# HybridRobotics/ilqr-iterative-tasks

Measured on AMD Instinct MI355X. Metric: batched iLQR iterations/s (n=6,m=2,N=20), higher is better.
Workload: dtype f64

## Files before the change

ilqr_iterative_tasks_amd/csrc/i2lqr_abi.hip:

```cpp
#include <hip/hip_runtime.h>

#include <atomic>
#include <cmath>
#include <cstdarg>
#include <cstdio>
#include <cstdlib>
#include <cstring>
#include <mutex>
#include <new>
#include <unordered_set>

#include "../../include/i2lqr.h"
#include "i2lqr_devcfg.hpp"
#include "i2lqr_geometry.hpp"
#include "i2lqr_group.h"
#include "i2lqr_host.hpp"
#include "i2lqr_kernels.h"
#include "i2lqr_lane12.h"
#include "i2lqr_rccl.hpp"
#include "i2lqr_select.hpp"
#include "i2lqr_wave_ls.h"
#include "i2lqr_wave_box.h"
#include "i2lqr_wave_obs.h"

// ... 107 lines not shown
                (long long)(rec & 0xfffffff));
  }
#else
  (void)stream;
#endif
  return rc;
}
}

struct i2lqr_handle {
  i2lqr_config cfg;
  int lanes;
  size_t lds_bytes;
  int device;
  void* ws = nullptr;
  int64_t ws_bytes = 0;
  int64_t compact_min_batch = -1;
  int opt_defer = -1, opt_reroll = -1, opt_lds_steps = -1, opt_merge = -1, opt_ckpt = -1, opt_stagger = -1;
  int wave_tail = -1;
  int opt_pair = -1;
  int opt_two_x = -1;
  int opt_chunk_step = -1;
  int opt_fuse = -1;
  int opt_final_round = -1;
  int opt_first_chunk = -1;
  int opt_fstep = -1;
  int opt_group = -1;
  int opt_spec = -1;
  int opt_group_ws = -1;
  int opt_group_overlap = -1;
  int opt_obs = 0;
  i2lqr::StateBox box;
  int opt_ls = 0;
  int opt_group_fixed = -1;
  struct Epilogue {
    const int32_t* qfun;
    int outer_iter, max_relax_iter;
    void* cost_it;
    void* part;
    int64_t* best_idx;
    void* best_cost;
    bool fused;
  };
  static constexpr unsigned kTickets = 16;
  unsigned* ticket = nullptr;
  std::atomic<unsigned> ticket_next{0};
  hipEvent_t ev_ready = nullptr, ev_side_done = nullptr;
  bool side_pending = false;
  DeviceGeometry geo;
};

namespace {
thread_local i2lqr_handle::Epilogue* t_epi = nullptr;
}

namespace {

enum FusedKernel { K_WAVE, K_WAVE_LS, K_WAVE_OBS, K_WAVE_BOX, K_GROUP, K_GROUP16, K_GROUP_WS, K_SPEC, K_SPEC16, K_QUAD, K_INVALID };
constexpr int64_t kAutoGroupBatch = 1024;
constexpr int64_t kAutoSpecBatch = 12288;

FusedKernel select_fused(const i2lqr_handle* h, int64_t B, bool early_exit, const char** why) {
  static const char* none = "";
  if (!why) why = &none;
  if (h->box.on()) {
    if (h->opt_group == 8 || h->opt_group == 16) {
// ... 110 lines not shown
  static constexpr int n = Sys::n, m = Sys::m, LANES = 64;
  using Cfg = DevCfg<T, n, m>;

  static size_t lds_bytes(int N) { return (size_t)Layout<Sys>(N).total * sizeof(T) * (64 / LANES); }
  static size_t fstep_lds_bytes(int N) {
    return (size_t)Layout<Sys>(N, true).total * sizeof(T) * (64 / LANES);
  }
  static constexpr bool kHasFstep = Sys::n <= 6;
  static unsigned grid(int64_t B) { return (unsigned)((B + (64 / LANES) - 1) / (64 / LANES)); }

  static int prepare(i2lqr_handle* h) {
    h->lanes = LANES;
    h->lds_bytes = lds_bytes(h->cfg.N);
    if (h->lds_bytes > h->geo.max_dyn_lds)
      return fail(I2LQR_ERR_UNSUPPORTED, "horizon %d needs %zu B of LDS per wavefront (> %zu KiB)",
                  h->cfg.N, h->lds_bytes, h->geo.max_dyn_lds / 1024);
    if (h->lds_bytes > h->geo.default_dyn_lds)
      for (const void* kernel :
           {(const void*)k_iterate<T, Sys, LANES, false>, (const void*)k_iterate<T, Sys, LANES, true>,
            (const void*)k_backward<T, Sys, LANES, false>, (const void*)k_backward<T, Sys, LANES, true>,
            (const void*)k_forward<T, Sys, LANES, false>, (const void*)k_forward<T, Sys, LANES, true>,
            (const void*)k_rollout<T, Sys, LANES, false>, (const void*)k_rollout<T, Sys, LANES, true>})
        HIP_TRY(hipFuncSetAttribute(kernel, hipFuncAttributeMaxDynamicSharedMemorySize,
                                    (int)h->lds_bytes));
    return I2LQR_OK;
  }

  static int iterate(i2lqr_handle* h, int64_t B, int n_iters, int early_exit, void* X, void* U,
                     const void* x_term, void* lamb, const void* obs, void* cost, void* K, void* k,
                     int32_t* iters, int32_t* status, hipStream_t s) {
    const Cfg c = make_dev_cfg<T, n, m>(h->cfg);
    IterArgs<T> a = iter_args<T>(B, n_iters, early_exit, X, U, x_term, lamb, obs, cost, K, k, iters,
                                 status);
#ifdef I2LQR_STAMPS
    a.dbg = (unsigned long long*)h->ws;
#endif
    const char* why = "";
    const FusedKernel fk = select_fused(h, B, early_exit != 0, &why);
    if (t_epi && (fk == K_GROUP || fk == K_GROUP16 || fk == K_GROUP_WS)) {
      a.qfun = t_epi->qfun;
      a.outer_iter = t_epi->outer_iter;
      a.max_relax_iter = t_epi->max_relax_iter;
      a.cost_it = (T*)t_epi->cost_it;
      if (t_epi->best_idx) {
        a.pick_part = (MinPair<T>*)t_epi->part;
        a.pick_ticket = h->ticket + h->ticket_next.fetch_add(1, std::memory_order_relaxed) %
                                        i2lqr_handle::kTickets;
        a.best_idx = t_epi->best_idx;
        a.best_cost = (T*)t_epi->best_cost;
      }
      t_epi->fused = true;
    }
    switch (fk) {
      case K_INVALID:
        return fail(I2LQR_ERR_UNSUPPORTED, "%s", why);
      case K_SPEC:
      case K_SPEC16:
        if constexpr (m == 2 && n + m <= 8) {
          HIP_TRY(group_spec_iterate<T>(h->cfg, a, s, fk == K_SPEC16 ? 16 : 8));
          return I2LQR_OK;
        }
        break;
      case K_GROUP:
        if constexpr (m == 2 && n + m <= 8) {
          HIP_TRY(group_iterate<T>(h->cfg, a, s));
          return I2LQR_OK;
// ... 48 lines not shown
    const int64_t waves_per_cu = (grid(B) + h->geo.cus - 1) / h->geo.cus;
    const bool fstep = kHasFstep && lds_f <= h->geo.default_dyn_lds &&
                       (h->opt_fstep >= 0 ? h->opt_fstep != 0
                                          : waves_per_cu * lds_f <= h->geo.lds_per_cu - 10 * 1024);
    if constexpr (kHasFstep) {
      if (fstep) {
        with_weights(c.flags, [&](auto W) {
          hipLaunchKernelGGL((k_iterate<T, Sys, LANES, W, true>), dim3(grid(B)), dim3(64), lds_f, s, c, a);
        });
        HIP_TRY(hipGetLastError());
        return I2LQR_OK;
      }
    }
    with_weights(c.flags, [&](auto W) {
      hipLaunchKernelGGL((k_iterate<T, Sys, LANES, W>), dim3(grid(B)), dim3(64), h->lds_bytes, s, c, a);
    });
    HIP_TRY(hipGetLastError());
    return I2LQR_OK;
  }
  static int names_pair(i2lqr_handle*, int64_t, int) { return 0; }
  static int solve_chained(i2lqr_handle* h, int64_t L, int k, void* X, void* U, const void* x_term,
                           void* lamb, const void* obs, void* cost, void* K, void* kk, int32_t* iters,
                           int32_t* status, hipStream_t s) {
    if constexpr (m == 2 && n + m <= 8) {
      if (h->opt_spec == 0 || h->opt_group == 8 || h->opt_group == 64 ||
          !group_spec_chain_supported(h->cfg, L))
        return fail(I2LQR_ERR_UNSUPPORTED, "chains run on the sixteen-lane speculative kernel: a "
                    "bicycle plant with Q = R = 0, at most %lld chains, a horizon whose three-wavefront "
                    "buffers fit a CU's LDS (solve the chain steps one after the other instead)",
                    (long long)h->geo.scaled(512));
      IterArgs<T> a = iter_args<T>(L, h->cfg.max_iter, 1, X, U, x_term, lamb, obs, cost, K, kk, iters,
                                   status);
      a.chain_len = k;
      HIP_TRY(group_spec_chain<T>(h->cfg, a, s));
      return I2LQR_OK;
    }
    return fail(I2LQR_ERR_UNSUPPORTED, "chains are built for the m = 2 plants");
  }
  static int rollout(i2lqr_handle* h, int64_t B, void* X, void* U, const void* x_term, void* cost,
                     hipStream_t s) {
    const Cfg c = make_dev_cfg<T, n, m>(h->cfg);
    with_weights(c.flags, [&](auto W) {
      hipLaunchKernelGGL((k_rollout<T, Sys, LANES, W>), dim3(grid(B)), dim3(64), h->lds_bytes, s, c,
                         B, (T*)X, (T*)U, (const T*)x_term, (T*)cost);
    });
    HIP_TRY(hipGetLastError());
    return I2LQR_OK;
  }
  static int backward(i2lqr_handle* h, int64_t B, const void* X, const void* U, const void* x_term,
                      const void* lamb, const void* obs, void* K, void* k, hipStream_t s) {
    const Cfg c = make_dev_cfg<T, n, m>(h->cfg);
    with_weights(c.flags, [&](auto W) {
      hipLaunchKernelGGL((k_backward<T, Sys, LANES, W>), dim3(grid(B)), dim3(64), h->lds_bytes, s, c,
                         B, (const T*)X, (const T*)U, (const T*)x_term, (const T*)lamb,
                         (const T*)obs, (T*)K, (T*)k);
    });
    HIP_TRY(hipGetLastError());
    return I2LQR_OK;
  }
  static int forward(i2lqr_handle* h, int64_t B, const void* X, const void* U, const void* x_term,
                     const void* K, const void* k, void* Xn, void* Un, void* cost_new,
                     hipStream_t s) {
    const Cfg c = make_dev_cfg<T, n, m>(h->cfg);
    with_weights(c.flags, [&](auto W) {
      hipLaunchKernelGGL((k_forward<T, Sys, LANES, W>), dim3(grid(B)), dim3(64), h->lds_bytes, s, c,
                         B, (const T*)X, (const T*)U, (const T*)x_term, (const T*)K, (const T*)k,
// ... 248 lines not shown
      a.cp.user_tiled = TILED ? 1 : 0;
      a.cp.orig = orig;
      if (dst) a.cp.dst = *dst;
      a.cp.count_out = count_out;
      a.cp.usr = usr;
    };
    int round = 0;
    int cur = 0;
    const bool only_chunk = len >= max_iter;
    plan_exit(a0, true, nullptr, only_chunk ? nullptr : &cv.set[cur], cv.count + round);
    launch_iterate<TILED>(h->geo, c, a0, B, s, h->opt_pair);
    done += len;
    const unsigned cgrid = (unsigned)((B + 255) / 256);
    bool src_user = true;
    const int32_t* count_in = nullptr;
    LaneSet<T> src = usr;
    const int final_round = (!spec_tail || wave_tail <= 0) ? 0
        : (h->opt_final_round >= 0 ? h->opt_final_round : kFinalRound);
    while (done < max_iter) {
      int32_t* const count = cv.count + round;
      if (!fused)
        hipLaunchKernelGGL((k_lane_compact<T, TILED>), dim3(cgrid), dim3(256), 0, s, n, m, N, src,
                           src_user ? 1 : 0, count_in, cv.set[cur], count, usr, c.trap);
      const LaneSet<T>& w = cv.set[cur];
      const bool tail_ran = wave_tail > 0 && done >= 4;
      const bool last_round = final_round > 0 && round + 1 >= final_round && tail_ran;
      if (tail_ran) {
        using WL = Launch<T, Sys>;
        const size_t lds_f = WL::fstep_lds_bytes(N);
        IterArgs<T> t = iter_args<T>(B, max_iter, 1, w.X, w.U, w.x_term, w.lamb, w.obs, w.cost, w.K,
                                     w.k, w.iters, w.status);
        t.count = count; t.count_max = last_round ? (int)B : wave_tail; t.max_total = max_iter;
        t.set_stride = B;
        if (spec_tail) {
          t.orig = w.orig;
          t.out_X = usr.X; t.out_U = usr.U; t.out_K = usr.K; t.out_k = usr.k;
          t.out_lamb = usr.lamb; t.out_cost = usr.cost;
          t.out_iters = usr.iters; t.out_status = usr.status;
          t.out_B = usr.B; t.out_tiled = TILED ? 1 : 0;
          if constexpr (m == 2 && n + m <= 8) HIP_TRY(group_spec_tail<T>(h->cfg, t, s));
        } else if (WL::kHasFstep && lds_f <= h->geo.default_dyn_lds) {
          if constexpr (WL::kHasFstep) {
            with_weights(c.flags, [&](auto W) {
              hipLaunchKernelGGL((k_iterate<T, Sys, 64, W, true, true>), dim3(wave_tail), dim3(64),
                                 lds_f, s, c, t);
            });
          }
        }
      }
      if (last_round && spec_tail && tail_ran) {
        src_user = true;
        break;
      }
      len = done < 12 ? step : done;
      if (done + len > max_iter || round + 2 >= kMaxRounds) len = max_iter - done;
      LaneArgs<T> a = a0;
      set_io(a, len, 1, w);
      a.K = nullptr; a.k = nullptr;
      a.count = count; a.resume = 1;
      plan_exit(a, false, w.orig, done + len >= max_iter ? nullptr : &cv.set[cur ^ 1],
                cv.count + round + 1);
      LaneArgs<T> ap = a;
      ap.ckpt = 0;
      ap.merge = h->opt_merge >= 0 ? h->opt_merge : 0;
      ap.reroll = h->opt_reroll >= 0 ? h->opt_reroll : 0;
      const unsigned pair_max = pair_max_grid(h->geo);
// ... 506 lines not shown
  return B % 64 == 0 ? I2LQR_LAYOUT_BATCH_TILED : I2LQR_LAYOUT_BATCH_MINOR;
}

int i2lqr_set_compaction(i2lqr_handle* h, int64_t min_batch) {
  if (!h) return fail(I2LQR_ERR_INVALID, "null handle");
  if (h->cfg.layout == I2LQR_LAYOUT_PROBLEM_MAJOR && min_batch > 0)
    return fail(I2LQR_ERR_UNSUPPORTED, "compaction applies to the batch-minor / batch-tiled layouts");
  h->compact_min_batch = min_batch < 0 ? -1 : min_batch;
  return I2LQR_OK;
}

int i2lqr_set_option(i2lqr_handle* h, const char* name, int64_t value) {
  if (!h || !name) return fail(I2LQR_ERR_INVALID, "null handle or option name");
  if (value < -1 || value > 0x7fffffff) return fail(I2LQR_ERR_INVALID, "option value out of range");
  const int v = (int)value;
  if (!strcmp(name, "defer_states")) h->opt_defer = v < 0 ? -1 : (v != 0);
  else if (!strcmp(name, "reroll_nominal")) h->opt_reroll = v < 0 ? -1 : (v != 0);
  else if (!strcmp(name, "lds_gain_steps")) h->opt_lds_steps = v;
  else if (!strcmp(name, "merge_inputs")) h->opt_merge = v < 0 ? -1 : (v != 0);
  else if (!strcmp(name, "checkpoint_states")) h->opt_ckpt = v < 0 ? -1 : (v != 0);
  else if (!strcmp(name, "stagger")) h->opt_stagger = v;
  else if (!strcmp(name, "per_step_jacobians")) h->opt_fstep = v < 0 ? -1 : (v != 0);
  else if (!strcmp(name, "wave_tail")) h->wave_tail = v < 0 ? -1 : (v > 65536 ? 65536 : v);
  else if (!strcmp(name, "first_chunk")) h->opt_first_chunk = v < 1 ? -1 : (v > 1024 ? 1024 : v);
  else if (!strcmp(name, "helper_wavefront")) h->opt_pair = v < 0 ? -1 : (v != 0);
  else if (!strcmp(name, "state_buffers")) h->opt_two_x = v < 0 ? -1 : (v != 0);
  else if (!strcmp(name, "chunk_step")) h->opt_chunk_step = v < 1 ? -1 : (v > 1024 ? 1024 : v);
  else if (!strcmp(name, "fused_compaction")) h->opt_fuse = v < 0 ? -1 : (v != 0);
  else if (!strcmp(name, "final_round")) h->opt_final_round = v < 0 ? -1 : (v > 20 ? 20 : v);
  else if (!strcmp(name, "speculate")) h->opt_spec = v < 0 ? -1 : (v != 0);
  else if (!strcmp(name, "group_workspace")) h->opt_group_ws = v < 0 ? -1 : (v != 0);
  else if (!strcmp(name, "group_overlap")) h->opt_group_overlap = v < 0 ? -1 : (v != 0);
  else if (!strcmp(name, "group_fixed_horizon")) h->opt_group_fixed = v < 0 ? -1 : (v != 0);
  else if (!strcmp(name, "debug_self_test")) {
#ifdef I2LQR_DEBUG
    unsigned long long* w = i2lqr::debug_trap_word();
    double* buf = nullptr;
    HIP_TRY(hipMalloc((void**)&buf, 8 * sizeof(double)));
    hipLaunchKernelGGL(k_debug_self_test, dim3(1), dim3(64), 0, (hipStream_t)0, buf, w);
    const int rc = debug_check(I2LQR_OK, nullptr);
    (void)hipFree(buf);
    return rc;
#else
    return fail(I2LQR_ERR_UNSUPPORTED, "\"debug_self_test\" exists in the index-checked debug build "
                "only (make -C ilqr_iterative_tasks_amd/csrc debug)");
#endif
  }
  else if (!strcmp(name, "line_search")) {
    if (v != -1 && v != 0 && v != 1 && v != 2 && v != 4 && v != 8)
      return fail(I2LQR_ERR_INVALID, "\"line_search\" is 2, 4 or 8 step sizes, or -1 / 0 / 1 (off)");
    if (v > 1 && h->cfg.layout != I2LQR_LAYOUT_PROBLEM_MAJOR)
      return fail(I2LQR_ERR_UNSUPPORTED, "\"line_search\" is built for the problem-major layout (the "
                  "one-problem-per-wavefront kernel)");
    h->opt_ls = v > 1 ? v : 0;
  }
  else if (!strcmp(name, "obstacles")) {
    if (v > I2LQR_MAX_OBSTACLES)
      return fail(I2LQR_ERR_INVALID, "\"obstacles\" is 2 ... %d records per problem, or -1 / 0 / 1 "
                  "(off: one record)", I2LQR_MAX_OBSTACLES);
    if (v > 1 && h->cfg.layout != I2LQR_LAYOUT_PROBLEM_MAJOR)
      return fail(I2LQR_ERR_UNSUPPORTED, "\"obstacles\" is built for the problem-major layout (the "
                  "one-problem-per-wavefront kernel)");
    h->opt_obs = v > 1 ? v : 0;
  }
  else if (!strcmp(name, "group_lanes")) {
    if (v != -1 && v != 8 && v != 16 && v != 64)
// ... 619 lines not shown
```

ilqr_iterative_tasks_amd/csrc/i2lqr_group.hpp:

```cpp
#pragma once
#include <hip/hip_runtime.h>
#include <stdint.h>

#include "i2lqr_systems.hpp"
#include "i2lqr_wave.hpp"

namespace i2lqr {

constexpr int kGroup = 8;
constexpr int kGroupsPerWave = 64 / kGroup;

template <class Sys> struct GroupPattern {
  static constexpr int n = Sys::n, m = Sys::m, W = n + m, NV = Sys::NVAR;
  static constexpr int dt_row(int b) {
    for (int i = 2; i < n; i++)
      if (i != b && Sys::pat(i, b) == 2) return i;
    return -1;
  }
  static constexpr bool column_ok(int b) {
    int extra = 0;
    for (int i = 0; i < n; i++) {
      const int code = Sys::pat(i, b);
      if (i < 2) {
        if (code == 2) return false;
// ... 215 lines not shown
      const T f = code == 2 ? c.dt : jv[code >= 3 ? code - 3 : 0];
      acc = first ? f * v : t_fma(f, v, acc);
      first = false;
    }
  }

  __device__ __forceinline__ T rollout(int XUo, int TRo, const T (&xT)[n]) const {
    T x[n], u[m], xn[n], tr[NT];
#pragma unroll
    for (int i = 0; i < n; i++) x[i] = S[XUo + i];
    const int N = loop_N();
    for (int t = 0; t < N; t++) {
#pragma unroll
      for (int a = 0; a < m; a++) u[a] = clip(S[XUo + t * W + n + a], -c.u_max[a], c.u_max[a]);
#pragma unroll
      for (int a = 0; a < m; a++) S[XUo + t * W + n + a] = u[a];
      Sys::trig(x, tr);
#pragma unroll
      for (int q = 0; q < NT; q++) S[TRo + t * NT + q] = tr[q];
      Sys::step_tr(c, x, u, tr, xn);
#pragma unroll
      for (int i = 0; i < n; i++) S[XUo + (t + 1) * W + i] = xn[i];
#pragma unroll
      for (int i = 0; i < n; i++) x[i] = xn[i];
    }
    Sys::trig(x, tr);
#pragma unroll
    for (int q = 0; q < NT; q++) S[TRo + N * NT + q] = tr[q];
    const T cost = terminal_cost(x, xT);
    wave_sync();
    return cost;
  }

  __device__ __forceinline__ void prep(int XUo, int TRo, const T (&ob)[6], T pa, T pb, int first,
                                       int stride) const {
    const bool has_ob = ob[5] >= T(0);
    const int opt = has_ob ? (int)ob[5] : 0;
    const T spd_y = opt == 1 ? ob[4] : T(0), spd_x = opt == 2 ? ob[4] : T(0);
    const int rounds = (N + stride) / stride;
    for (int r = 0; r < rounds; r++) {
      const int t0 = first + r * stride;
      const int t = t0 < N ? t0 : N;
      const int ts = t0 < N ? t0 : N - 1;
      T* Rs = rec(ts);
      {
        T xe[n], tr[NT], u[m], jv[NV];
#pragma unroll
        for (int i = 0; i < n; i++) xe[i] = S[XUo + (ts + 1) * W + i];
#pragma unroll
        for (int a = 0; a < m; a++) u[a] = S[XUo + ts * W + n + a];
#pragma unroll
        for (int q = 0; q < NT; q++) tr[q] = S[TRo + (ts + 1) * NT + q];
        Sys::jac_var(c, xe, u, tr, jv);
#pragma unroll
        for (int q = 0; q < NV; q++) Rs[GL::R_JV + q] = jv[q];
#pragma unroll
        for (int a = 0; a < m; a++) {
          T e_hi, e_lo;
          if (sizeof(T) == 8 && c.fast_barrier) {
            e_hi = t_exp_bounded(c.ctrl_q2 * (u[a] - c.u_max[a]));
            e_lo = c.ctrl_c[a] * t_rcp(e_hi);
          } else {
            e_hi = t_exp(c.ctrl_q2 * (u[a] - c.u_max[a]));
            e_lo = t_exp(c.ctrl_q2 * (-c.u_max[a] - u[a]));
          }
          Rs[GL::R_LU + a] = c.ctrl_q12 * e_hi - c.ctrl_q12 * e_lo;
          Rs[GL::R_LUU + a] = c.ctrl_q122 * e_hi +
                              c.ctrl_q122 * e_lo;
        }
      }
      T* R = rec(t);
      R[GL::R_ZERO] = T(0);
      R[GL::R_ONE] = T(1);
      const T px = S[XUo + t * W + 0], py = S[XUo + t * W + 1];
      const T dz = opt == 2 ? px - (ob[0] - T(t) * spd_x) : px - ob[0];
      const T dy = opt == 1 ? py - (ob[1] + T(t) * spd_y) : py - ob[1];
      const T h = T(1) + c.safety_margin - (dz * pa * dz + dy * pb * dy);
      const T hd0 = T(-2) * pa * dz, hd1 = T(-2) * pb * dy;
      const T e = t_exp(c.obs_q2 * h);
      const T c1 = c.obs_q12 * e, c2 = c.obs_q122 * e;
      R[GL::R_OB + 0] = has_ob ? c1 * hd0 : T(0);
      R[GL::R_OB + 1] = has_ob ? c1 * hd1 : T(0);
      R[GL::R_OB + 2] = has_ob ? c2 * (hd0 * hd0) : T(0);
      R[GL::R_OB + 3] = has_ob ? c2 * (hd0 * hd1) : T(0);
      R[GL::R_OB + 4] = has_ob ? c2 * (hd1 * hd1) : T(0);
    }
    wave_sync();
    ws_publish();
  }

  __device__ __forceinline__ void quu_inverse(const T (&Quu)[m * m], T lamb, T (&inv)[m * m]) const {
    static_assert(m == 2, "the eight-lane kernel is written for m == 2 plants");
    t_quu_inverse2(Quu, lamb, inv);
  }

  template <bool GENERAL>
  __device__ __forceinline__ bool backward(int XUo, const T (&xT)[n], T lamb, bool commit) const {
    if constexpr (G == 16) return backward_row<GENERAL>(XUo, xT, lamb, commit);
    bool bad = false;
    T va[n];
    {
      const T* Rn = rec(N);
      T dx[n];
#pragma unroll
      for (int i = 0; i < n; i++) dx[i] = S[XUo + N * W + i] - xT[i];
#pragma unroll
      for (int i = 0; i < n; i++) {
        T vxx = T(0), vx = T(0);
#pragma unroll
        for (int r = 0; r < n; r++) {
          const T q = T(2) * Qt[i * n + r];
          vxx = (g == r) ? q : vxx;
          vx += q * dx[r];
        }
        va[i] = (g == n) ? vx : vxx;
      }
      va[0] += Rn[off_l0];
      va[1] += Rn[off_l1];
// ... 114 lines not shown
        for (int b = 0; b < m; b++) acc = t_fma(Quu[a * m + b], kc[b], acc);
        qk[a] = acc;
      }
#pragma unroll
      for (int i = 0; i < n; i++) {
        T acc = T(0);
#pragma unroll
        for (int a = 0; a < m; a++) acc = t_fma(kr[a][i], qk[a], acc);
        va[i] = h[i] - acc;
      }
      STAMP_END(5);
    };
    int t = N - 1;
    if constexpr (I2LQR_GROUP_UNROLL >= 4) {
      for (; t >= 3; t -= 4) {
        step(t, ra, rb);
        step(t - 1, rb, ra);
        step(t - 2, ra, rb);
        step(t - 3, rb, ra);
      }
    }
    for (; t >= 1; t -= 2) {
      step(t, ra, rb);
      step(t - 1, rb, ra);
    }
    if (t == 0) step(0, ra, rb);
    ws_publish();
    return bad;
  }

  template <bool GENERAL>
  __device__ __forceinline__ bool backward_row(int XUo, const T (&xT)[n], T lamb, bool commit) const {
    T vb[n];
    terminal_base(XUo, xT, vb);
    return backward_row_from<GENERAL>(vb, lamb, commit);
  }
  __device__ __forceinline__ void terminal_base(int XUo, const T (&xT)[n], T (&vb)[n]) const {
    T dx[n];
#pragma unroll
    for (int i = 0; i < n; i++) dx[i] = S[XUo + N * W + i] - xT[i];
    const int gq = g < n ? g : 0;
#pragma unroll
    for (int i = 0; i < n; i++) {
      T vx = T(0);
#pragma unroll
      for (int r = 0; r < n; r++) vx += (T(2) * Qt[i * n + r]) * dx[r];
      const T vxx = T(2) * Qt[i * n + gq];
      vb[i] = (g == n) ? vx : (g < n ? vxx : T(0));
    }
  }
  template <bool GENERAL>
  __device__ __forceinline__ bool backward_row_from(const T (&vb)[n], T lamb, bool commit) const {
    static_assert(GL::KW > n + 1, "the padding word of a gain row takes the stores of idle lanes");
    bool bad = false;
    T va[n];
    {
      const T* Rn = rec(N);
#pragma unroll
      for (int i = 0; i < n; i++) va[i] = vb[i];
      va[0] += Rn[off_l0];
      va[1] += Rn[off_l1];
    }
    const int gcol = (commit && g <= n) ? g : GL::KW - 1;
    T cdr[n];
#pragma unroll
    for (int r = 0; r < n; r++) cdr[r] = (rsrc == r) ? cdt : T(0);
    struct Rec { T jv[NV], luu[m], c0, c1, l0, l1, lrow[m]; };
    Rec ra, rb;
    constexpr bool FIXED = NH > 0 && !GENERAL;
    const T* const R0 = rec(0);
    const T *pc0 = R0, *pc1 = R0, *pl0 = R0, *pl1 = R0, *plu[m];
#pragma unroll
    for (int a = 0; a < m; a++) plu[a] = R0;
    if constexpr (FIXED) {
      pc0 = R0 + off_c0; pc1 = R0 + off_c1; pl0 = R0 + off_l0; pl1 = R0 + off_l1;
#pragma unroll
      for (int a = 0; a < m; a++) plu[a] = R0 + off_lu[a];
    }
    auto load_record = [&](int t, Rec& r) __attribute__((always_inline)) {
      if constexpr (FIXED) {
        const int o = t * GL::RW;
// ... 317 lines not shown
  }
};

__device__ __forceinline__ int idx_div(int e, int d, float rcp_d) {
  int q = (int)((float)e * rcp_d);
  const int r = e - q * d;
  q += (r >= d) ? 1 : 0;
  q -= (r < 0) ? 1 : 0;
  return q;
}

template <class T, class Sys, int H, bool WS, int G, int NH>
__device__ __forceinline__ void group_iterate_body(const DevCfg<T, Sys::n, Sys::m>& c,
                                                   const IterArgs<T>& a, T* ws) {
  static_assert(!(WS && H > 1), "the workspace form runs without helper wavefronts");
  constexpr int n = Sys::n, m = Sys::m, W = n + m;
#ifdef I2LQR_STAMPS
  constexpr bool OVL = false;
#else
  constexpr bool OVL = G == 16 && H >= 3;
#endif
  using GL = GLayout<Sys, G>;
  extern __shared__ __align__(16) unsigned char gsmem_raw[];
  T* smem = reinterpret_cast<T*>(gsmem_raw);
  const int lane = threadIdx.x & 63, hv = threadIdx.x >> 6;
#ifdef I2LQR_STAMPS
  unsigned long long st_k0, st_k1, st_k2, st_k3;
  asm volatile("s_memtime %0\n\ts_waitcnt lgkmcnt(0)" : "=s"(st_k0)::"memory");
#endif
  const int64_t prob0 = (int64_t)blockIdx.x * GL::PW + lane / G;
  const bool real = prob0 < a.B;
  const int64_t prob = real ? prob0 : a.B - 1;
  GroupWorker<T, Sys, WS, G, NH> w(c, smem, lane);
  const int N = NH > 0 ? NH : c.N, g = w.g;
  const float rN = 1.0f / (float)N, rN1 = 1.0f / (float)(N + 1), rnN = 1.0f / (float)(n * N);
  const GL& L = w.L;
  const auto S = w.S;
  if constexpr (WS) w.Wp = ws + prob0 * (int64_t)L.ws_words();

  if (H == 1 || hv == 0) {
    const T* gX = a.X + prob * (int64_t)(n * (N + 1));
    if (g < n) S[L.XU0 + g] = gX[g * (N + 1)];
    const T* gU = a.U + prob * (int64_t)(m * N);
    for (int e = g; e < m * N; e += G) {
      const int aa = idx_div(e, N, rN), t = e - aa * N;
      S[L.XU0 + t * W + n + aa] = gU[e];
    }
    for (int e = lane; e < n * n; e += 64) smem[L.qt_base() + e] = c.Qt[e];
  }
  T xT[n], ob[6];
#pragma unroll
  for (int i = 0; i < n; i++) xT[i] = a.x_term[prob * n + i];
#pragma unroll
  for (int q = 0; q < 6; q++) ob[q] = a.obs ? a.obs[prob * 6 + q] : T(q == 5 ? -1 : 1);
  T lamb = a.lamb[prob];
  wave_sync();

  int cur = 0;
  const T ob_pa = T(1) / (ob[2] * ob[2]), ob_pb = T(1) / (ob[3] * ob[3]);
  int* const ctl = reinterpret_cast<int*>(smem + L.ctl_base());
  if constexpr (H > 1) {
    if (hv > 0) {
      const int h0 = OVL ? hv - 1 : hv, hs = OVL ? H - 1 : H;
      for (;;) {
        __syncthreads();
        const int flags = ctl[8];
        if (!(flags & 1)) break;
        if (flags & 2) {
          const int pc = ctl[lane / G];
          w.prep(pc ? L.XU1 : L.XU0, pc ? L.TR1 : L.TR0, ob, ob_pa, ob_pb, h0 * G + g, hs * G);
        }
        __syncthreads();
      }
      if constexpr (OVL) {
        if (real && a.K) {
          T* const gK = a.K + prob * (int64_t)(m * n * N);
          T* const gk = a.k + prob * (int64_t)(m * N);
          for (int t = h0 * G + g; t < N; t += hs * G) {
            const T* Kt = w.gain(t);
            T kv[m][n + 1];
#pragma unroll
            for (int aa = 0; aa < m; aa++)
#pragma unroll
              for (int j = 0; j <= n; j++) kv[aa][j] = Kt[aa * GL::KW + j];
#pragma unroll
            for (int aa = 0; aa < m; aa++) {
#pragma unroll
              for (int j = 0; j < n; j++) gK[(aa * n + j) * N + t] = kv[aa][j];
              gk[aa * N + t] = kv[aa][n];
            }
          }
        }
      }
      return;
    }
  }
  T vb[n];
#pragma unroll
  for (int i = 0; i < n; i++) vb[i] = T(0);
  T cost = w.rollout(L.XU0, L.TR0, xT);
  int it = 0, status = a.early_exit ? 2  : 0 ;
  T cost_ret = cost;
  bool fresh = true, active = a.n_iters > 0;
#ifdef I2LQR_STAMPS
  asm volatile("s_memtime %0\n\ts_waitcnt lgkmcnt(0)" : "=s"(st_k1)::"memory");
#endif
  while (__any(active)) {
    const int XUo = cur ? L.XU1 : L.XU0, XUn = cur ? L.XU0 : L.XU1;
    const int TRo = cur ? L.TR1 : L.TR0, TRn = cur ? L.TR0 : L.TR1;
#ifdef I2LQR_STAMPS
    {
      auto& st_t0 = w.st_t0; auto& st_t1 = w.st_t1; auto& st_acc = w.st_acc;
      STAMP_BEGIN();
      if (__any(fresh)) w.prep(XUo, TRo, ob, ob_pa, ob_pb, g, G);
      STAMP_END(0);
    }
#else
    if constexpr (H > 1) {
      const bool do_prep = __any(fresh);
      if (g == 0) ctl[lane / G] = cur;
      if (lane == 0) ctl[8] = 1 | (do_prep ? 2 : 0);
      __syncthreads();
      if constexpr (OVL) {
        if (do_prep) w.terminal_base(XUo, xT, vb);
      } else {
        if (do_prep) w.prep(XUo, TRo, ob, ob_pa, ob_pb, g, H * G);
      }
      __syncthreads();
    } else {
      if (__any(fresh)) w.prep(XUo, TRo, ob, ob_pa, ob_pb, g, G);
    }
#endif
    if constexpr (OVL) {
      if (__builtin_expect(__any(w.template backward_row_from<false>(vb, lamb, active)), 0))
        w.template backward_row_from<true>(vb, lamb, active);
    } else {
      if (__builtin_expect(__any(w.template backward<false>(XUo, xT, lamb, active)), 0))
        w.template backward<true>(XUo, xT, lamb, active);
    }
    T cost_new;
    {
#ifdef I2LQR_STAMPS
      auto& st_t0 = w.st_t0; auto& st_t1 = w.st_t1; auto& st_acc = w.st_acc;
      STAMP_BEGIN();
#endif
      bool big = false;
      cost_new = w.template forward<false>(XUo, XUn, TRn, xT, &big);
      if (__builtin_expect(__any(big), 0)) cost_new = w.template forward<true>(XUo, XUn, TRn, xT, &big);
#ifdef I2LQR_STAMPS
      STAMP_END(6);
#endif
    }
    {
      const bool acc = active && cost_new < cost, rej = active && !(cost_new < cost);
      const T lamb_dn = lamb / c.lamb_factor, lamb_up = lamb * c.lamb_factor;
      const bool conv = t_abs((cost_new - cost) / cost) < c.eps;
      it += active ? 1 : 0;
      fresh = acc;
      cur ^= acc ? 1 : 0;
      lamb = acc ? lamb_dn : (rej ? lamb_up : lamb);
      cost_ret = acc ? cost_new : (rej ? cost : cost_ret);
      cost = acc ? cost_new : cost;
      const bool stop_conv = acc && conv, stop_lamb = rej && lamb > c.max_lamb;
// ... 134 lines not shown
  __host__ __device__ int group_words() const { return PW * total + n * n + (V + 1) * PW; }
};

template <class T, class Sys, int V, bool SETIO = false, int G = kGroup, bool CHAIN = false>
__global__ __launch_bounds__(64 * V) void k_group_spec(const DevCfg<T, Sys::n, Sys::m> c,
                                                       const IterArgs<T> a) {
  static_assert(!(CHAIN && SETIO), "chains are problem-major batches");
  constexpr int n = Sys::n, m = Sys::m, W = n + m;
  using GL = GLayout<Sys, G>;
  using SL = GSpecLayout<Sys, V, G>;
  constexpr int PW = SL::PW;
  extern __shared__ __align__(16) unsigned char gsmem_raw[];
  T* smem = reinterpret_cast<T*>(gsmem_raw);
  const int v = threadIdx.x >> 6, lane = threadIdx.x & 63;
  const int p = lane / G, g = lane % G;
  const int64_t prob0 = (int64_t)blockIdx.x * PW + p;
  int64_t live = a.B;
  if constexpr (SETIO) {
    live = *a.count;
    if (live > a.count_max || (int64_t)blockIdx.x * PW >= live) return;
  }
  const int64_t Bs = SETIO ? a.set_stride : 0;
  const bool real = prob0 < live;
  const int clen = CHAIN ? a.chain_len : 1;
  T lamb_carry = T(0);
 for (int cstep = 0; cstep < clen; cstep++) {
  const int64_t prob = CHAIN ? (real ? prob0 : live - 1) * clen + cstep : (real ? prob0 : live - 1);
  const SL SLay(c.N);
  const int N = c.N;
  T* const S = smem + p * SLay.total;
  T* const QtL = smem + PW * SLay.total;
  T* const CN = QtL + n * n;
  GroupWorker<T, Sys, false, G> w(c, S, QtL, g, SLay.total);
  w.oR = SLay.R;
  w.oKk = SLay.var0 + v * SLay.var_words + SLay.Kk_in_var;
  if constexpr (G == kGroup) w.T1c = S + SLay.var0 + v * SLay.var_words + SLay.T1c_in_var;

  if (v == 0) {
    if constexpr (SETIO) {
      if (g < n) S[SLay.xu_off(0) + g] = a.X[g * Bs + prob];
      for (int e = g; e < m * N; e += G) {
        const int t = e / m, aa = e - t * m;
        S[SLay.xu_off(0) + t * W + n + aa] = a.U[e * Bs + prob];
      }
    } else {
      const T* gX = a.X + prob * (int64_t)(n * (N + 1));
      if (g < n) S[SLay.xu_off(0) + g] = gX[g * (N + 1)];
      const T* gU = a.U + prob * (int64_t)(m * N);
      for (int e = g; e < m * N; e += G) {
        const int aa = e / N, t = e - aa * N;
        S[SLay.xu_off(0) + t * W + n + aa] = gU[e];
      }
    }
    for (int e = lane; e < n * n; e += 64) QtL[e] = c.Qt[e];
  }
  T xT[n], ob[6];
#pragma unroll
  for (int i = 0; i < n; i++) xT[i] = SETIO ? a.x_term[i * Bs + prob] : a.x_term[prob * n + i];
#pragma unroll
  for (int q = 0; q < 6; q++)
    ob[q] = a.obs ? (SETIO ? a.obs[q * Bs + prob] : a.obs[prob * 6 + q]) : T(q == 5 ? -1 : 1);
  T lamb = (CHAIN && cstep > 0) ? lamb_carry : a.lamb[prob];
  const int it0 = SETIO ? a.iters[prob] : 0;
  const int it_cap = SETIO ? a.max_total - it0 : a.n_iters;
  const T ob_pa = T(1) / (ob[2] * ob[2]), ob_pb = T(1) / (ob[3] * ob[3]);
  __syncthreads();
  if (v == 0) {
    const T c0 = w.rollout(SLay.xu_off(0), SLay.tr_off(0), xT);
    if (g == 0) CN[V * PW + p] = c0;
  }
  __syncthreads();
  T cost = CN[V * PW + p];

  int nb = 0, cb[V];
#pragma unroll
  for (int k = 0; k < V; k++) cb[k] = k + 1;
  int it = 0, status = a.early_exit ? 2  : 0 , gsel = 0;
  T cost_ret = cost;
  bool fresh = true, active = it_cap > 0;
  while (__any(active)) {
    if (__any(fresh)) {
      w.prep(SLay.xu_off(nb), SLay.tr_off(nb), ob, ob_pa, ob_pb, v * G + g, V * G);
      __syncthreads();
    }
    T lamb_v = lamb;
    for (int k = 0; k < v; k++) lamb_v *= c.lamb_factor;
    int mycb = cb[0];
#pragma unroll
    for (int k = 1; k < V; k++) mycb = (v == k) ? cb[k] : mycb;
    const int XUo = SLay.xu_off(nb), XUn = SLay.xu_off(mycb), TRn = SLay.tr_off(mycb);
    if (__builtin_expect(__any(w.template backward<false>(XUo, xT, lamb_v, active)), 0))
      w.template backward<true>(XUo, xT, lamb_v, active);
    bool big = false;
    T cost_new = w.template forward<false>(XUo, XUn, TRn, xT, &big);
    if (__builtin_expect(__any(big), 0)) cost_new = w.template forward<true>(XUo, XUn, TRn, xT, &big);
    if (g == 0) CN[v * PW + p] = cost_new;
    __syncthreads();
    fresh = false;
    bool chain = active;
#pragma unroll
    for (int k = 0; k < V; k++) {
      if (chain) {
        const T cn = CN[k * PW + p];
        it++;
        gsel = k;
        if (cn < cost) {
          const int tb = nb; nb = cb[k]; cb[k] = tb;
          lamb /= c.lamb_factor;
          const bool conv = t_abs((cn - cost) / cost) < c.eps;
          cost_ret = cn;
          cost = cn;
          fresh = true;
          chain = false;
          if (conv) {
            if (a.early_exit) { status = 1; active = false; }
// ... 100 lines not shown
```

ilqr_iterative_tasks_amd/csrc/i2lqr_systems.hpp:

```cpp
#pragma once
#include <hip/hip_runtime.h>

#include <type_traits>

namespace i2lqr {

template <class T> __device__ __forceinline__ void t_sincos(T x, T* s, T* c);
template <bool SLIT, unsigned long long BITS>
__device__ __forceinline__ double t_lit_at(double dep) {
  if constexpr (SLIT) {
    unsigned lo, hi;
    asm volatile("s_mov_b32 %0, %2\n\ts_mov_b32 %1, %3"
                 : "=s"(lo), "=s"(hi)
                 : "n"((unsigned)(BITS & 0xffffffffull)), "n"((unsigned)(BITS >> 32)), "v"(dep));
    return __builtin_bit_cast(double, ((unsigned long long)hi << 32) | lo);
  } else {
    return __builtin_bit_cast(double, BITS);
  }
}
#define I2LQR_LIT(SLIT, value, dep) \
  t_lit_at<SLIT, __builtin_bit_cast(unsigned long long, (double)(value))>(dep)
template <class T> __device__ __forceinline__ void t_sincos_fast(T x, T* s, T* c, bool* big_out);
template <bool SLIT, int NS>
__device__ __forceinline__ void t_sincos_fast_dn(const double (&x)[NS], double (&s)[NS],
// ... 173 lines not shown
  for (int q = 0; q < NE; q++) p[q] = c13;
#define I2LQR_EXP_STEP(lit)                                          \
  {                                                                  \
    const double ck = I2LQR_LIT(SLIT, lit, p[0]);                    \
    _Pragma("unroll") for (int q = 0; q < NE; q++) p[q] = __builtin_fma(p[q], r[q], ck); \
  }
  I2LQR_EXP_STEP(2.0876756987868098979e-09)
  I2LQR_EXP_STEP(2.5052108385441718775e-08)
  I2LQR_EXP_STEP(2.7557319223985890653e-07)
  I2LQR_EXP_STEP(2.7557319223985892511e-06)
  I2LQR_EXP_STEP(2.4801587301587301566e-05)
  I2LQR_EXP_STEP(1.9841269841269841253e-04)
  I2LQR_EXP_STEP(1.3888888888888889419e-03)
  I2LQR_EXP_STEP(8.3333333333333332177e-03)
  I2LQR_EXP_STEP(4.1666666666666664354e-02)
  I2LQR_EXP_STEP(1.6666666666666665741e-01)
#undef I2LQR_EXP_STEP
#pragma unroll
  for (int q = 0; q < NE; q++) {
    p[q] = __builtin_fma(p[q], r[q], 0.5);
    p[q] = __builtin_fma(p[q], r[q], 1.0);
    p[q] = __builtin_fma(p[q], r[q], 1.0);
    const double v = __builtin_ldexp(p[q], (int)kf[q]);
    e[q] = q < NE - NB ? (x0[q] < I2LQR_LIT(SLIT, -745.14, v) ? 0.0
                          : (x0[q] > I2LQR_LIT(SLIT, 709.79, v) ? __builtin_inf() : v))
                       : v;
  }
}
template <> __device__ __forceinline__ double t_exp<double>(double x0) {
  const double xa[1] = {x0};
  double ea[1];
  t_exp_d<false, 1, 0>(xa, ea);
  return ea[0];
}
template <class T> __device__ __forceinline__ T t_exp_bounded(T x);
template <> __device__ __forceinline__ double t_exp_bounded<double>(double x) {
  const double xa[1] = {x};
  double ea[1];
  t_exp_d<false, 1, 1>(xa, ea);
  return ea[0];
}
template <> __device__ __forceinline__ float t_exp_bounded<float>(float x) { return __expf(x); }
template <> __device__ __forceinline__ float t_exp<float>(float x) { return __expf(x); }
template <class T> __device__ __forceinline__ T t_sqrt(T x);
template <> __device__ __forceinline__ double t_sqrt<double>(double x) { return sqrt(x); }
template <> __device__ __forceinline__ float t_sqrt<float>(float x) { return sqrtf(x); }
template <class T> __device__ __forceinline__ T t_abs(T x) { return x < T(0) ? -x : x; }
template <class T> __device__ __forceinline__ T t_fma(T a, T b, T c);
template <> __device__ __forceinline__ double t_fma<double>(double a, double b, double c) {
  return __builtin_fma(a, b, c);
}
template <> __device__ __forceinline__ float t_fma<float>(float a, float b, float c) {
  return __builtin_fmaf(a, b, c);
}

template <class T> __device__ __forceinline__ T t_rcp(T x);
template <> __device__ __forceinline__ double t_rcp<double>(double x) {
  double r = __builtin_amdgcn_rcp(x);
  double e = __builtin_fma(-x, r, 1.0);
  r = __builtin_fma(r, e, r);
  e = __builtin_fma(-x, r, 1.0);
  const double r2 = __builtin_fma(r, e, r);
  return (r2 == r2) ? r2 : r;
}
template <> __device__ __forceinline__ float t_rcp<float>(float x) {
  const float r = __builtin_amdgcn_rcpf(x);
// ... 597 lines not shown
```

ilqr_iterative_tasks_amd/csrc/i2lqr_wave.hpp:

```cpp
#pragma once
#include <hip/hip_runtime.h>
#include <stdint.h>

#include <type_traits>

#include "i2lqr_debug.hpp"
#include "i2lqr_systems.hpp"


namespace i2lqr {

enum : int { FLAG_HAS_Q = 1, FLAG_HAS_R = 2 };

template <class T, int n, int m> struct DevCfg {
  int N, max_iter, flags;
  int fast_barrier;
  T dt, eps, lamb_factor, max_lamb;
  T ctrl_q1, ctrl_q2, obs_q1, obs_q2, safety_margin;
  T u_max[m];
  T ctrl_c[m];
  T xtarget[n];
  T Q[n * n], Qt[n * n], R[m * m];
  T sys_par[8];
  T ctrl_q12, ctrl_q122, obs_q12, obs_q122;
// ... 18 lines not shown
  T* X;
  T* U;
  const T* x_term;
  T* lamb;
  const T* obs;
  T* cost;
  T* K;
  T* k;
  int32_t* iters;
  int32_t* status;
  unsigned long long* dbg;
  const int32_t* count;
  int count_max, max_total;
  int64_t set_stride;
  const int32_t* orig = nullptr;
  T* out_X = nullptr;
  T* out_U = nullptr;
  T* out_K = nullptr;
  T* out_k = nullptr;
  T* out_lamb = nullptr;
  T* out_cost = nullptr;
  int32_t* out_iters = nullptr;
  int32_t* out_status = nullptr;
  int64_t out_B = 0;
  int out_tiled = 0;
  const int32_t* qfun = nullptr;
  int outer_iter = 0, max_relax_iter = 0;
  T* cost_it = nullptr;
  MinPair<T>* pick_part = nullptr;
  unsigned* pick_ticket = nullptr;
  int64_t* best_idx = nullptr;
  T* best_cost = nullptr;
  int chain_len = 1;
};

__device__ __forceinline__ double relax_cost_value(double ss, int32_t qf, int N, int outer_iter,
                                                   int max_relax_iter) {
  const double nrm = sqrt(ss);
  double scale = 1.0;
  for (int q = 0; q < outer_iter; q++) scale *= 10.0;
  double out = INFINITY;
  if (qf == 0x7fffffff) return out;
  for (int i = 1; i <= max_relax_iter; i++) {
    if (nrm <= 80.0 * i / scale) { out = (double)qf + N + 100 * i; break; }
    if (nrm > 80.0 * max_relax_iter / scale) break;
  }
  return out;
}

template <class T>
__device__ __forceinline__ void pick_epilogue(const IterArgs<T>& a, bool cand, int64_t prob, T v) {
  T bv = cand ? v : T(0);
  int64_t bi = (cand && v == v) ? prob : -1;
#pragma unroll
  for (int s = 32; s > 0; s >>= 1) {
    const T ov = __shfl_xor(bv, s);
    const int64_t oi = __shfl_xor(bi, s);
    if (oi >= 0 && better(ov, oi, bv, bi)) { bv = ov; bi = oi; }
  }
  const int lane = threadIdx.x & 63;
  unsigned ticket = 0;
  if (lane == 0) {
    __hip_atomic_store(&a.pick_part[blockIdx.x].v, bv, __ATOMIC_RELAXED, __HIP_MEMORY_SCOPE_AGENT);
    __hip_atomic_store(&a.pick_part[blockIdx.x].i, bi, __ATOMIC_RELAXED, __HIP_MEMORY_SCOPE_AGENT);
    __threadfence();
    ticket = atomicInc(a.pick_ticket, gridDim.x - 1);
// ... 834 lines not shown
```

Baseline: 82.19 million.

## Batch barrier exponentials in group prep and broadcast terminal value gradient

Splits the group-kernel record preparation into a fast path that evaluates the obstacle and control-bound exponentials together in one vectorised exp call with clamped arguments, and a general path. The terminal base computes one gradient entry per lane and broadcasts it with cross-lane moves instead of every lane computing all n dot products. The helper-wave loop reads its control flag uniformly with readfirstlane, and a new option selects the fast prep path. This aims to cut transcendental and ALU work in prep, at the cost of an extra barrier in the helper loop and slightly different exp clamping behaviour.

```diff
diff --git a/ilqr_iterative_tasks_amd/csrc/i2lqr_abi.hip b/ilqr_iterative_tasks_amd/csrc/i2lqr_abi.hip
--- a/ilqr_iterative_tasks_amd/csrc/i2lqr_abi.hip
+++ b/ilqr_iterative_tasks_amd/csrc/i2lqr_abi.hip
@@ -163,6 +163,7 @@
   int opt_obs = 0;
   i2lqr::StateBox box;
   int opt_ls = 0;
+  int opt_group_records = -1;
   int opt_group_fixed = -1;
   struct Epilogue {
     const int32_t* qfun;
@@ -339,6 +340,7 @@
     const Cfg c = make_dev_cfg<T, n, m>(h->cfg);
     IterArgs<T> a = iter_args<T>(B, n_iters, early_exit, X, U, x_term, lamb, obs, cost, K, k, iters,
                                  status);
+    a.group_records = h->opt_group_records != 0;
 #ifdef I2LQR_STAMPS
     a.dbg = (unsigned long long*)h->ws;
 #endif
@@ -453,6 +455,7 @@
       IterArgs<T> a = iter_args<T>(L, h->cfg.max_iter, 1, X, U, x_term, lamb, obs, cost, K, kk, iters,
                                    status);
       a.chain_len = k;
+      a.group_records = h->opt_group_records != 0;
       HIP_TRY(group_spec_chain<T>(h->cfg, a, s));
       return I2LQR_OK;
     }
@@ -767,6 +770,7 @@
                                      w.k, w.iters, w.status);
         t.count = count; t.count_max = last_round ? (int)B : wave_tail; t.max_total = max_iter;
         t.set_stride = B;
+        t.group_records = h->opt_group_records != 0;
         if (spec_tail) {
           t.orig = w.orig;
           t.out_X = usr.X; t.out_U = usr.U; t.out_K = usr.K; t.out_k = usr.k;
@@ -1339,6 +1343,10 @@
   else if (!strcmp(name, "group_workspace")) h->opt_group_ws = v < 0 ? -1 : (v != 0);
   else if (!strcmp(name, "group_overlap")) h->opt_group_overlap = v < 0 ? -1 : (v != 0);
   else if (!strcmp(name, "group_fixed_horizon")) h->opt_group_fixed = v < 0 ? -1 : (v != 0);
+  else if (!strcmp(name, "group_records")) {
+    if (v > 1) return fail(I2LQR_ERR_INVALID, "\"group_records\" is 0, 1 or -1");
+    h->opt_group_records = v;
+  }
   else if (!strcmp(name, "debug_self_test")) {
 #ifdef I2LQR_DEBUG
     unsigned long long* w = i2lqr::debug_trap_word();
diff --git a/ilqr_iterative_tasks_amd/csrc/i2lqr_group.hpp b/ilqr_iterative_tasks_amd/csrc/i2lqr_group.hpp
--- a/ilqr_iterative_tasks_amd/csrc/i2lqr_group.hpp
+++ b/ilqr_iterative_tasks_amd/csrc/i2lqr_group.hpp
@@ -271,58 +271,118 @@
     return cost;
   }
 
+  __device__ __forceinline__ void prep_fast(int XUo, int TRo, const T (&ob)[6], T pa, T pb,
+                                            bool has_ob, int opt, T spd_x, T spd_y, int t,
+                                            int ts) const {
+    T xe[n], tr[NT], u[m], jv[NV];
+#pragma unroll
+    for (int i = 0; i < n; i++) xe[i] = S[XUo + (ts + 1) * W + i];
+#pragma unroll
+    for (int a = 0; a < m; a++) u[a] = S[XUo + ts * W + n + a];
+#pragma unroll
+    for (int q = 0; q < NT; q++) tr[q] = S[TRo + (ts + 1) * NT + q];
+    const T px = S[XUo + t * W + 0], py = S[XUo + t * W + 1];
+    Sys::jac_var(c, xe, u, tr, jv);
+    const T dz = opt == 2 ? px - (ob[0] - T(t) * spd_x) : px - ob[0];
+    const T dy = opt == 1 ? py - (ob[1] + T(t) * spd_y) : py - ob[1];
+    const T h = T(1) + c.safety_margin - (dz * pa * dz + dy * pb * dy);
+    const T hd0 = T(-2) * pa * dz, hd1 = T(-2) * pb * dy;
+    double ea[m + 1], ee[m + 1];
+    const double eo = c.obs_q2 * h;
+    ea[0] = t_exp_sel_arg(eo);
+#pragma unroll
+    for (int a = 0; a < m; a++) ea[1 + a] = c.ctrl_q2 * (u[a] - c.u_max[a]);
+    t_exp_d<false, m + 1, m + 1>(ea, ee);
+    ee[0] = t_exp_sel_end(eo, ee[0]);
+    T e_lo[m];
+#pragma unroll
+    for (int a = 0; a < m; a++) e_lo[a] = c.ctrl_c[a] * t_rcp(T(ee[1 + a]));
+    const T c1 = c.obs_q12 * T(ee[0]), c2 = c.obs_q122 * T(ee[0]);
+    T* Rs = rec(ts);
+    T* R = rec(t);
+#pragma unroll
+    for (int q = 0; q < NV; q++) Rs[GL::R_JV + q] = jv[q];
+#pragma unroll
+    for (int a = 0; a < m; a++) {
+      const T e_hi = T(ee[1 + a]);
+      Rs[GL::R_LU + a] = c.ctrl_q12 * e_hi - c.ctrl_q12 * e_lo[a];
+      Rs[GL::R_LUU + a] = c.ctrl_q122 * e_hi +
+                          c.ctrl_q122 * e_lo[a];
+    }
+    R[GL::R_ZERO] = T(0);
+    R[GL::R_ONE] = T(1);
+    R[GL::R_OB + 0] = has_ob ? c1 * hd0 : T(0);
+    R[GL::R_OB + 1] = has_ob ? c1 * hd1 : T(0);
+    R[GL::R_OB + 2] = has_ob ? c2 * (hd0 * hd0) : T(0);
+    R[GL::R_OB + 3] = has_ob ? c2 * (hd0 * hd1) : T(0);
+    R[GL::R_OB + 4] = has_ob ? c2 * (hd1 * hd1) : T(0);
+  }
+
+  __device__ __forceinline__ void prep_general(int XUo, int TRo, const T (&ob)[6], T pa, T pb,
+                                               bool has_ob, int opt, T spd_x, T spd_y, int t,
+                                               int ts) const {
+    T* Rs = rec(ts);
+    {
+      T xe[n], tr[NT], u[m], jv[NV];
+#pragma unroll
+      for (int i = 0; i < n; i++) xe[i] = S[XUo + (ts + 1) * W + i];
+#pragma unroll
+      for (int a = 0; a < m; a++) u[a] = S[XUo + ts * W + n + a];
+#pragma unroll
+      for (int q = 0; q < NT; q++) tr[q] = S[TRo + (ts + 1) * NT + q];
+      Sys::jac_var(c, xe, u, tr, jv);
+#pragma unroll
+      for (int q = 0; q < NV; q++) Rs[GL::R_JV + q] = jv[q];
+      T e_hi[m], e_lo[m];
+#pragma unroll
+      for (int a = 0; a < m; a++) e_hi[a] = t_exp_sel(c.ctrl_q2 * (u[a] - c.u_max[a]));
+#pragma unroll
+      for (int a = 0; a < m; a++) e_lo[a] = c.ctrl_c[a] * t_rcp(e_hi[a]);
+      if (!(sizeof(T) == 8 && c.fast_barrier)) {
+#pragma unroll
+        for (int a = 0; a < m; a++) e_lo[a] = t_exp_sel(c.ctrl_q2 * (-c.u_max[a] - u[a]));
+      }
+#pragma unroll
+      for (int a = 0; a < m; a++) {
+        Rs[GL::R_LU + a] = c.ctrl_q12 * e_hi[a] - c.ctrl_q12 * e_lo[a];
+        Rs[GL::R_LUU + a] = c.ctrl_q122 * e_hi[a] +
+                            c.ctrl_q122 * e_lo[a];
+      }
+    }
+    T* R = rec(t);
+    R[GL::R_ZERO] = T(0);
+    R[GL::R_ONE] = T(1);
+    const T px = S[XUo + t * W + 0], py = S[XUo + t * W + 1];
+    const T dz = opt == 2 ? px - (ob[0] - T(t) * spd_x) : px - ob[0];
+    const T dy = opt == 1 ? py - (ob[1] + T(t) * spd_y) : py - ob[1];
+    const T h = T(1) + c.safety_margin - (dz * pa * dz + dy * pb * dy);
+    const T hd0 = T(-2) * pa * dz, hd1 = T(-2) * pb * dy;
+    const T e = t_exp_sel(c.obs_q2 * h);
+    const T c1 = c.obs_q12 * e, c2 = c.obs_q122 * e;
+    R[GL::R_OB + 0] = has_ob ? c1 * hd0 : T(0);
+    R[GL::R_OB + 1] = has_ob ? c1 * hd1 : T(0);
+    R[GL::R_OB + 2] = has_ob ? c2 * (hd0 * hd0) : T(0);
+    R[GL::R_OB + 3] = has_ob ? c2 * (hd0 * hd1) : T(0);
+    R[GL::R_OB + 4] = has_ob ? c2 * (hd1 * hd1) : T(0);
+  }
+
   __device__ __forceinline__ void prep(int XUo, int TRo, const T (&ob)[6], T pa, T pb, int first,
-                                       int stride) const {
+                                       int stride, bool lean) const {
     const bool has_ob = ob[5] >= T(0);
     const int opt = has_ob ? (int)ob[5] : 0;
     const T spd_y = opt == 1 ? ob[4] : T(0), spd_x = opt == 2 ? ob[4] : T(0);
     const int rounds = (N + stride) / stride;
+    const bool fast = sizeof(T) == 8 && c.fast_barrier && lean;
     for (int r = 0; r < rounds; r++) {
       const int t0 = first + r * stride;
       const int t = t0 < N ? t0 : N;
       const int ts = t0 < N ? t0 : N - 1;
-      T* Rs = rec(ts);
-      {
-        T xe[n], tr[NT], u[m], jv[NV];
-#pragma unroll
-        for (int i = 0; i < n; i++) xe[i] = S[XUo + (ts + 1) * W + i];
-#pragma unroll
-        for (int a = 0; a < m; a++) u[a] = S[XUo + ts * W + n + a];
-#pragma unroll
-        for (int q = 0; q < NT; q++) tr[q] = S[TRo + (ts + 1) * NT + q];
-        Sys::jac_var(c, xe, u, tr, jv);
-#pragma unroll
-        for (int q = 0; q < NV; q++) Rs[GL::R_JV + q] = jv[q];
-#pragma unroll
-        for (int a = 0; a < m; a++) {
-          T e_hi, e_lo;
-          if (sizeof(T) == 8 && c.fast_barrier) {
-            e_hi = t_exp_bounded(c.ctrl_q2 * (u[a] - c.u_max[a]));
-            e_lo = c.ctrl_c[a] * t_rcp(e_hi);
-          } else {
-            e_hi = t_exp(c.ctrl_q2 * (u[a] - c.u_max[a]));
-            e_lo = t_exp(c.ctrl_q2 * (-c.u_max[a] - u[a]));
-          }
-          Rs[GL::R_LU + a] = c.ctrl_q12 * e_hi - c.ctrl_q12 * e_lo;
-          Rs[GL::R_LUU + a] = c.ctrl_q122 * e_hi +
-                              c.ctrl_q122 * e_lo;
-        }
-      }
-      T* R = rec(t);
-      R[GL::R_ZERO] = T(0);
-      R[GL::R_ONE] = T(1);
-      const T px = S[XUo + t * W + 0], py = S[XUo + t * W + 1];
-      const T dz = opt == 2 ? px - (ob[0] - T(t) * spd_x) : px - ob[0];
-      const T dy = opt == 1 ? py - (ob[1] + T(t) * spd_y) : py - ob[1];
-      const T h = T(1) + c.safety_margin - (dz * pa * dz + dy * pb * dy);
-      const T hd0 = T(-2) * pa * dz, hd1 = T(-2) * pb * dy;
-      const T e = t_exp(c.obs_q2 * h);
-      const T c1 = c.obs_q12 * e, c2 = c.obs_q122 * e;
-      R[GL::R_OB + 0] = has_ob ? c1 * hd0 : T(0);
-      R[GL::R_OB + 1] = has_ob ? c1 * hd1 : T(0);
-      R[GL::R_OB + 2] = has_ob ? c2 * (hd0 * hd0) : T(0);
-      R[GL::R_OB + 3] = has_ob ? c2 * (hd0 * hd1) : T(0);
-      R[GL::R_OB + 4] = has_ob ? c2 * (hd1 * hd1) : T(0);
+      if constexpr (sizeof(T) == 8) {
+        if (fast) prep_fast(XUo, TRo, ob, pa, pb, has_ob, opt, spd_x, spd_y, t, ts);
+        else prep_general(XUo, TRo, ob, pa, pb, has_ob, opt, spd_x, spd_y, t, ts);
+      } else {
+        prep_general(XUo, TRo, ob, pa, pb, has_ob, opt, spd_x, spd_y, t, ts);
+      }
     }
     wave_sync();
     ws_publish();
@@ -503,7 +563,9 @@
   template <bool GENERAL>
   __device__ __forceinline__ bool backward_row(int XUo, const T (&xT)[n], T lamb, bool commit) const {
     T vb[n];
+    STAMP_BEGIN();
     terminal_base(XUo, xT, vb);
+    STAMP_END(5);
     return backward_row_from<GENERAL>(vb, lamb, commit);
   }
   __device__ __forceinline__ void terminal_base(int XUo, const T (&xT)[n], T (&vb)[n]) const {
@@ -511,13 +573,25 @@
 #pragma unroll
     for (int i = 0; i < n; i++) dx[i] = S[XUo + N * W + i] - xT[i];
     const int gq = g < n ? g : 0;
+    T qrow[n], qcol[n];
+#pragma unroll
+    for (int r = 0; r < n; r++) qrow[r] = Qt[gq * n + r];
+#pragma unroll
+    for (int i = 0; i < n; i++) qcol[i] = Qt[i * n + gq];
+#pragma unroll
+    for (int i = 0; i < n; i++) asm("" : "+v"(qcol[i]));
+    T vx = T(0);
+#pragma unroll
+    for (int r = 0; r < n; r++) vx += (T(2) * qrow[r]) * dx[r];
+    T vxs[n];
+    static_for_i<0, n>([&](auto i_) {
+      constexpr int i = decltype(i_)::value;
+      vxs[i] = bcast_mov<i>(vx);
+    });
 #pragma unroll
     for (int i = 0; i < n; i++) {
-      T vx = T(0);
-#pragma unroll
-      for (int r = 0; r < n; r++) vx += (T(2) * Qt[i * n + r]) * dx[r];
-      const T vxx = T(2) * Qt[i * n + gq];
-      vb[i] = (g == n) ? vx : (g < n ? vxx : T(0));
+      const T vxx = T(2) * qcol[i];
+      vb[i] = (g == n) ? vxs[i] : (g < n ? vxx : T(0));
     }
   }
   template <bool GENERAL>
@@ -901,6 +975,7 @@
   const bool real = prob0 < a.B;
   const int64_t prob = real ? prob0 : a.B - 1;
   GroupWorker<T, Sys, WS, G, NH> w(c, smem, lane);
+  const bool lean = a.group_records != 0;
   const int N = NH > 0 ? NH : c.N, g = w.g;
   const float rN = 1.0f / (float)N, rN1 = 1.0f / (float)(N + 1), rnN = 1.0f / (float)(n * N);
   const GL& L = w.L;
@@ -931,15 +1006,16 @@
   if constexpr (H > 1) {
     if (hv > 0) {
       const int h0 = OVL ? hv - 1 : hv, hs = OVL ? H - 1 : H;
-      for (;;) {
-        __syncthreads();
-        const int flags = ctl[8];
-        if (!(flags & 1)) break;
+      __syncthreads();
+      int flags = __builtin_amdgcn_readfirstlane(ctl[8]);
+      while (flags & 1) {
         if (flags & 2) {
           const int pc = ctl[lane / G];
-          w.prep(pc ? L.XU1 : L.XU0, pc ? L.TR1 : L.TR0, ob, ob_pa, ob_pb, h0 * G + g, hs * G);
+          w.prep(pc ? L.XU1 : L.XU0, pc ? L.TR1 : L.TR0, ob, ob_pa, ob_pb, h0 * G + g, hs * G, lean);
         }
         __syncthreads();
+        __syncthreads();
+        flags = __builtin_amdgcn_readfirstlane(ctl[8]);
       }
       if constexpr (OVL) {
         if (real && a.K) {
@@ -981,7 +1057,7 @@
     {
       auto& st_t0 = w.st_t0; auto& st_t1 = w.st_t1; auto& st_acc = w.st_acc;
       STAMP_BEGIN();
-      if (__any(fresh)) w.prep(XUo, TRo, ob, ob_pa, ob_pb, g, G);
+      if (__any(fresh)) w.prep(XUo, TRo, ob, ob_pa, ob_pb, g, G, lean);
       STAMP_END(0);
     }
 #else
@@ -993,11 +1069,11 @@
       if constexpr (OVL) {
         if (do_prep) w.terminal_base(XUo, xT, vb);
       } else {
-        if (do_prep) w.prep(XUo, TRo, ob, ob_pa, ob_pb, g, H * G);
+        if (do_prep) w.prep(XUo, TRo, ob, ob_pa, ob_pb, g, H * G, lean);
       }
       __syncthreads();
     } else {
-      if (__any(fresh)) w.prep(XUo, TRo, ob, ob_pa, ob_pb, g, G);
+      if (__any(fresh)) w.prep(XUo, TRo, ob, ob_pa, ob_pb, g, G, lean);
     }
 #endif
     if constexpr (OVL) {
@@ -1198,6 +1274,7 @@
   T* const QtL = smem + PW * SLay.total;
   T* const CN = QtL + n * n;
   GroupWorker<T, Sys, false, G> w(c, S, QtL, g, SLay.total);
+  const bool lean = a.group_records != 0;
   w.oR = SLay.R;
   w.oKk = SLay.var0 + v * SLay.var_words + SLay.Kk_in_var;
   if constexpr (G == kGroup) w.T1c = S + SLay.var0 + v * SLay.var_words + SLay.T1c_in_var;
@@ -1246,7 +1323,7 @@
   bool fresh = true, active = it_cap > 0;
   while (__any(active)) {
     if (__any(fresh)) {
-      w.prep(SLay.xu_off(nb), SLay.tr_off(nb), ob, ob_pa, ob_pb, v * G + g, V * G);
+      w.prep(SLay.xu_off(nb), SLay.tr_off(nb), ob, ob_pa, ob_pb, v * G + g, V * G, lean);
       __syncthreads();
     }
     T lamb_v = lamb;
diff --git a/ilqr_iterative_tasks_amd/csrc/i2lqr_systems.hpp b/ilqr_iterative_tasks_amd/csrc/i2lqr_systems.hpp
--- a/ilqr_iterative_tasks_amd/csrc/i2lqr_systems.hpp
+++ b/ilqr_iterative_tasks_amd/csrc/i2lqr_systems.hpp
@@ -229,6 +229,21 @@
   double ea[1];
   t_exp_d<false, 1, 0>(xa, ea);
   return ea[0];
+}
+__device__ __forceinline__ double t_exp_sel_arg(double x0) {
+  const double lo = x0 < -746.0 ? -746.0 : x0;
+  return lo > 710.0 ? 710.0 : lo;
+}
+__device__ __forceinline__ double t_exp_sel_end(double x0, double v) {
+  const double hi = x0 > 709.79 ? __builtin_inf() : v;
+  return x0 < -745.14 ? 0.0 : hi;
+}
+template <class T> __device__ __forceinline__ T t_exp_sel(T x) { return t_exp(x); }
+template <> __device__ __forceinline__ double t_exp_sel<double>(double x0) {
+  const double xa[1] = {t_exp_sel_arg(x0)};
+  double ea[1];
+  t_exp_d<false, 1, 1>(xa, ea);
+  return t_exp_sel_end(x0, ea[0]);
 }
 template <class T> __device__ __forceinline__ T t_exp_bounded(T x);
 template <> __device__ __forceinline__ double t_exp_bounded<double>(double x) {
diff --git a/ilqr_iterative_tasks_amd/csrc/i2lqr_wave.hpp b/ilqr_iterative_tasks_amd/csrc/i2lqr_wave.hpp
--- a/ilqr_iterative_tasks_amd/csrc/i2lqr_wave.hpp
+++ b/ilqr_iterative_tasks_amd/csrc/i2lqr_wave.hpp
@@ -74,6 +74,7 @@
   int64_t* best_idx = nullptr;
   T* best_cost = nullptr;
   int chain_len = 1;
+  int group_records = 1;
 };
 
 __device__ __forceinline__ double relax_cost_value(double ss, int32_t qf, int N, int outer_iter,
```

Measured after the change: 82.06 million. About the same (-0.2%).
